# rvp-group/srrg2_proslam

Hardware: AMD Instinct MI355X
Metric: tracked frames/sec on KITTI-00 stereo (1241x376, ~2k kp); SE(3) vs ref (higher is better)
Workload: dtype u64 popcount (Hamming) + f32 (projection, Jacobians, 6x6 normal equations)

## Files before the change

srrg2_proslam_amd/csrc/align.hip:

```cpp
#include "prs_device.h"
#include "prs_host.h"
#include "prs_se3.h"

#include <math.h>
#include <string.h>

#include <type_traits>
#include <vector>

namespace prs {

constexpr int kAlignThreads = 256;
constexpr int kTerms        = 29;
constexpr uint32_t kNoneU32 = 0xffffffffu;
constexpr float kFltMax     = 3.402823466e+38f;

typedef unsigned int au32x4 __attribute__((ext_vector_type(4)));

struct AlignShared {
  float X[16];
  float A[16];
  float Sinv[16];
  float T[16];
  float Tprev[16];
// ... 971 lines not shown
          if (bind) {
            const uint32_t wsum = wave_inclusive_scan_dpp((uint32_t) msum), wabs = wave_inclusive_scan_dpp((uint32_t) mabs);
            const bool winexact = __ballot(inexact) != 0ull;
            if (lane == 63) {
              atomicAdd(&dsum[0], (int) wsum);
              atomicAdd(&dsum[1], (int) wabs);
              if (winexact) {
                dsum[2] = 1;
              }
            }
          }
          __syncthreads();
          if (sh.error) {
            break;
          }
          {
            const int chunk_r = (R + T) / T, chunk_c = (g.ncells + T) / T;
            uint32_t sum_r = 0, sum_c = 0;
            for (int j = 0; j < chunk_r; ++j) {
              const int r = tid * chunk_r + j;
              sum_r += r <= R ? hist_row[r] : 0u;
            }
            for (int j = 0; j < chunk_c; ++j) {
              const int r = tid * chunk_c + j;
              sum_c += r <= g.ncells ? hist_cell[r] : 0u;
            }
            const uint32_t incl_r = wave_inclusive_scan_dpp(sum_r), incl_c = wave_inclusive_scan_dpp(sum_c);
            if (lane == 63) {
              sh.wave_tot[wave]          = (int) incl_r;
              sh.wave_tot[kWaves + wave] = (int) incl_c;
            }
            if (bind && tid == T - 64) {
              const bool exact = !dsum[2] && dsum[1] < (1 << 24);
              const float acc  = exact ? (float) dsum[0] * 0.0625f : serial_float_sum(disp, nF);
              sh.mean_disp     = nF > 0 ? acc / (float) (size_t) nF : 0.0f;
            }
            __syncthreads();
            uint32_t run_r = incl_r - sum_r, run_c = incl_c - sum_c;
#pragma unroll
            for (int w = 0; w < kWaves; ++w) {
              run_r += w < wave ? (uint32_t) sh.wave_tot[w] : 0u;
              run_c += w < wave ? (uint32_t) sh.wave_tot[kWaves + w] : 0u;
            }
            for (int j = 0; j < chunk_r; ++j) {
              const int r = tid * chunk_r + j;
              if (r <= R) {
                rowfirst[r] = (uint16_t) run_r;
                run_r += hist_row[r];
              }
            }
            for (int j = 0; j < chunk_c; ++j) {
              const int r = tid * chunk_c + j;
              if (r <= g.ncells) {
                cellstart[r] = (uint16_t) run_c;
                run_c += hist_cell[r];
              }
            }
          }
          __syncthreads();
          for (int i = tid; i < nF; i += T) {
            bucket[rowfirst[rowcol[i] & 0xffffu] + slot[i]] = (uint16_t) i;
          }
          __syncthreads();
          for (int i = tid; i < nF; i += T) {
            const uint32_t rc = rowcol[i];
            const int row = (int) (rc & 0xffffu), col = (int) (rc >> 16);
            const int s = rowfirst[row], e = rowfirst[row + 1];
            int rank = 0;
            for (int j = s; j < e; ++j) {
              rank += bucket[j] < (uint16_t) i ? 1 : 0;
            }
            const int canon = s + rank;
            int cxi         = col >> g.cell_sx;
            cxi             = cxi < g.cell_ncx ? cxi : g.cell_ncx - 1;
            db[cellstart[(row >> g.cell_sy) * g.cell_ncx + cxi] + cslot[i]] = make_uint2(rc, (uint32_t) i | ((uint32_t) canon << 16));
            inv[canon]                                                      = (uint16_t) i;
          }
          if (tid == 0) {
            db[nF] = make_uint2(0x7fff7fffu, 0xffffffffu);
          }
          __syncthreads();
          db_built = true;
          if (split_search && g.dbcache) {
            const uint4* src = reinterpret_cast<const uint4*>(smem + g.off_db);
            uint4* dst       = reinterpret_cast<uint4*>(g.dbcache + (size_t) frame * g.db_blob);
            for (int i = tid; i < (int) (g.db_blob >> 4); i += T) {
              dst[i] = src[i];
            }
            if (tid == 0) {
              ctl->db_ready = 1;
            }
          }
        }

        SUB_ACC(acc_db);
        const int rad = (int) sh.radius;
        {
          const int tid = cold_copy(tid_hot);
          for (int i = tid; i < nF; i += T) {
            bestkey[i] = kNoneU32;
            second[i]  = kNoneU32;
          }
          if (lattice) {
            if (stage_rows) {
              au32x4* rows = split_search && g.rowcache ? g.rowcache + (size_t) frame * 2 * (size_t) g.max_fixed : nullptr;
              for (int pos = tid; pos < nF; pos += T) {
                const int fi    = (int) (db[pos].y & 0xffffu);
                const au32x4 lo = gfd[2 * fi], hi = gfd[2 * fi + 1];
                fdesc[pos]      = lo;
                fdesc_hi[pos]   = hi;
                if (rows) {
                  rows[pos]               = lo;
                  rows[g.max_fixed + pos] = hi;
                }
              }
            }
          } else {
            for (int i = tid; i < 2 * nF; i += T) {
              (i & 1 ? fdesc_hi : fdesc)[i >> 1] = gfd[i];
            }
            for (int i = tid; i < nF; i += T) {
              const float4 c = gfix[i];
              fuv[i]         = make_float2(c.x, c.y);
            }
          }
          if (stype == PRS_SEARCH_CIRCLE) {
            for (int i = tid; i < 2 * rad + 1 && i < g.lut_cap; i += T) {
              const int h = i - rad;
              lut[i]      = (uint16_t) (isqrt_exact(rad * rad - h * h) + 1);
            }
          }
        }
        __syncthreads();
        SUB_ACC(acc_pass2);
        {
          const float W0 = sh.W[0], W1 = sh.W[1], W2 = sh.W[2], W3 = sh.W[3];
          const float W4 = sh.W[4], W5 = sh.W[5], W6 = sh.W[6], W7 = sh.W[7];
          const float W8 = sh.W[8], W9 = sh.W[9], W10 = sh.W[10], W11 = sh.W[11];
          const float cols = (float) g.f.projector.canvas_cols, rows = (float) g.f.projector.canvas_rows;
          const float max_dd = g.f.maximum_descriptor_distance;
          const float r2f    = (float) (sh.radius * sh.radius);
          const int rad2     = rad * rad;
          const int irrelevant = irrelevant_distance(sh.dd, g.f.maximum_distance_ratio_to_second_best);
          const int prune_at   = (lattice && irrelevant > 0 && irrelevant <= 54 && !g.no_prefilter && !sh.no_prune) ? irrelevant : 0;
          const bool circle_exact = rad < 8192 && R + rad < 32000 && (g.cell_ncx << g.cell_sx) + rad < 32000;
          int projected      = 0;
          const bool q_on   = kReuse && split_search && g.qcache != nullptr && prune_at > 0;
          const int q_tag   = q_on ? (prune_at | ((prune_at <= g.narrow_prefilter_limit ? 3 : 4) << 8)) : 0;
          const bool q_read = q_on && (sh.q_tag & 0xffff) == q_tag;
          au32x4* const qc  = q_on ? g.qcache + mbase : nullptr;
          if (kReuse && split_search && tid == 0) {
            sh.q_tag = (sh.q_tag & 0xffff) | (q_tag << 16);
          }
          auto query = [&](const int m, const float4 p, au32x4 q0, au32x4 q1, auto first_pass_tag) {
            constexpr bool FIRST_PASS = decltype(first_pass_tag)::value;
            au32x4 ent = {0u, 0u, 0u, 0u};
            if (FIRST_PASS) {
              ent = qc[m];
            }
            const float x = ((W0 * p.x + W1 * p.y) + W2 * p.z) + W3;
            const float y = ((W4 * p.x + W5 * p.y) + W6 * p.z) + W7;
            const float z = ((W8 * p.x + W9 * p.y) + W10 * p.z) + W11;
            uint2 cd      = make_uint2(kNoneU32, kNoneU32);
            bool visible  = !(z < g.f.projector.range_min || z > g.f.projector.range_max);
            float u = 0.0f, v = 0.0f;
            if (visible) {
              const float hx = g.f.projector.fx * x + g.f.projector.cx * z;
              const float hy = g.f.projector.fy * y + g.f.projector.cy * z;
              u              = hx / z;
              v              = hy / z;
              visible        = !(u < 0.0f || u >= cols || v < 0.0f || v >= rows);
            }
            if (!FIRST_PASS && SPLIT && SLOTS == 4) {
              asm volatile("" : "+v"(q0), "+v"(q1));
            }
            if (visible) {
              if (!FIRST_PASS) {
                ++projected;
              }
              bool hit = false, cached = false;
              uint32_t bestk = kNoneU32, seck = kNoneU32;
              int row = 0, col = 0, rmin = 0, rmax = 0, cmin = 0, cmax = 0;
              int r0, r1, cb0, cb1;
              if (lattice) {
                row  = (int) (int16_t) roundf(v);
                col  = (int) (int16_t) roundf(u);
                rmin = (int) (int16_t) (row - rad);
                rmax = (int) (int16_t) (row + rad + 1);
                cmin = (int) (int16_t) (col - rad - 1);
                cmax = (int) (int16_t) (col + rad + 1);
                r0   = rmin;
                r1   = rmax - 1;
                cb0  = col - rad;
                cb1  = col + rad;
              } else {
                const KdNode* nodes        = reinterpret_cast<const KdNode*>(db);
                const uint16_t* leaf_start = cellstart + 2;
                int code                   = (int) reinterpret_cast<const short*>(cellstart)[0];
                while (code >= 0) {
                  const KdNode nd = nodes[code];
                  code            = (int) nd.child[kd_side(nd, u, v) < 0.0f ? 0 : 1];
                }
                const int leaf = ~code;
                for (int o = leaf_start[leaf]; o < (int) leaf_start[leaf + 1]; ++o) {
                  const int fi   = inv[o];
                  const float2 c = fuv[fi];
                  const float du = c.x - u, dv = c.y - v;
                  if (du * du + dv * dv < r2f) {
                    const uint32_t d   = (uint32_t) hamming_regs(fdesc[fi], fdesc_hi[fi], q0, q1);
                    const uint32_t key = (float) d < max_dd ? ((d << 16) | (uint32_t) fi) : kNoneU32;
                    bestk              = key < bestk ? key : bestk;
                  }
                }
                r0 = 1;
                r1 = cb0 = cb1 = 0;
              }
              r0  = (lattice && r0 < 0) ? 0 : r0;
              r1  = r1 > R - 1 ? R - 1 : r1;
              cb0 = cb0 < 0 ? 0 : cb0;
              const int colmax = (g.cell_ncx << g.cell_sx) - 1;
              cb1 = cb1 > colmax ? colmax : cb1;
              if (r0 <= r1 && cb0 <= cb1) {
                const int cx0 = cb0 >> g.cell_sx, cx1 = cb1 >> g.cell_sx;
                const uint32_t query_rc = ((uint32_t) row & 0xffffu) | ((uint32_t) col << 16);
                auto accepts_circle = [&](const uint2 e) -> bool {
                  typedef short i16x2 __attribute__((ext_vector_type(2)));
                  const i16x2 d = __builtin_bit_cast(i16x2, e.x) - __builtin_bit_cast(i16x2, query_rc);
                  return __builtin_amdgcn_sdot2(d, d, 0, false) <= rad2;
                };
                auto accepts_any = [&](const uint2 e) -> bool {
                  const int drow = (int) (int16_t) (e.x & 0xffffu);
                  const int dcol = (int) (int16_t) (e.x >> 16);
                  if (drow < rmin || drow >= rmax) {
                    return false;
                  } else if (stype == PRS_SEARCH_SQUARE) {
                    return dcol > cmin && dcol < cmax;
                  } else if (stype == PRS_SEARCH_CIRCLE) {
                    const int h     = drow - row;
                    const int li    = h + rad;
                    const int width = li < g.lut_cap ? (int) lut[li] : isqrt_exact(rad * rad - h * h) + 1;
                    return dcol > col - width && dcol < col + width;
                  } else {
                    int width = (int) (int16_t) (drow - rmin + 1);
                    if (width > (int) (int16_t) rad) {
                      width = (int) (int16_t) (rmax - drow);
                    }
                    return dcol > col - width && dcol < col + width;
                  }
                };
                const bool lean_circle = stype == PRS_SEARCH_CIRCLE && circle_exact;
                auto score_at = [&](const int p) {
                  const uint32_t ey = db[p].y;
                  const uint32_t d  = (uint32_t) hamming_regs(fdesc[p], fdesc_hi[p], q0, q1);
                  const uint32_t key = (d << 16) | (ey >> 16);
                  const uint32_t hi  = key > bestk ? key : bestk;
                  seck               = hi < seck ? hi : seck;
                  bestk              = key < bestk ? key : bestk;
                };
                typedef __attribute__((address_space(3))) unsigned char lds_byte;
                const uint32_t fd_lds = (uint32_t) (uintptr_t) (lds_byte*) fdesc;
                auto scan = [&](auto accepts, auto pruned_tag) {
                  constexpr int WORDS = decltype(pruned_tag)::value;
                  constexpr bool PRUNED = WORDS != 0;
                  const uint16_t* cs = cellstart + (r0 >> g.cell_sy) * g.cell_ncx + cx0;
                  const int width    = cx1 + 1 - cx0;
                  int rows_left      = (r1 >> g.cell_sy) - (r0 >> g.cell_sy) + 1;
                  int pos = 0, seg1 = 0;
                  int n_surv = 0;
                  for (;;) {
                    if (pos >= seg1) {
                      if (rows_left <= 0) {
                        break;
                      }
                      pos  = cs[0];
                      seg1 = cs[width];
                      cs += g.cell_ncx;
                      --rows_left;
                    }
                    if (pos < seg1) {
                      if (PRUNED) {
                        au32x4 la, lb;
                        asm volatile("ds_read_b128 %0, %2\n\tds_read_b128 %1, %2 offset:16\n\ts_waitcnt lgkmcnt(0)"
                                     : "=&v"(la), "=&v"(lb)
                                     : "v"(fd_lds + 16u * (uint32_t) pos));
                        const bool hit_a = (WORDS == 3 ? hamming_96(la, q0) : hamming_half(la, q0)) < prune_at;
                        const bool hit_b = (WORDS == 3 ? hamming_96(lb, q0) : hamming_half(lb, q0)) < prune_at;
                        if (hit_a) {
                          surv[n_surv & (kSurvivors - 1)] = (uint16_t) pos;
                          ++n_surv;
                        }
                        if (hit_b) {
                          surv[n_surv & (kSurvivors - 1)] = (uint16_t) (pos + 1);
                          ++n_surv;
                        }
                      } else {
                        const unsigned long long wa = reinterpret_cast<const unsigned long long*>(db)[pos];
                        const unsigned long long wb = reinterpret_cast<const unsigned long long*>(db)[pos + 1];
                        const uint2 ea = make_uint2((uint32_t) wa, (uint32_t) (wa >> 32)), eb = make_uint2((uint32_t) wb, (uint32_t) (wb >> 32));
                        const bool in_a = accepts(ea);
                        const bool in_b = (pos + 1 < seg1) & accepts(eb);
                        if (in_a) {
                          score_at(pos);
                        }
                        if (in_b) {
                          score_at(pos + 1);
                        }
                      }
                      pos += 2;
                    }
                  }
                  return n_surv;
                };
                auto scan_pattern = [&](auto pruned_tag) {
                  return lean_circle ? scan(accepts_circle, pruned_tag) : scan(accepts_any, pruned_tag);
                };
                auto settle = [&](const int n_surv) {
                  for (int i = 0; i < n_surv; ++i) {
                    const int p = (int) surv[i];
                    bool seen   = false;
                    for (int j = 0; j < i; ++j) {
                      seen = seen | ((int) surv[j] == p);
                    }
                    if (!seen && (lean_circle ? accepts_circle(db[p]) : accepts_any(db[p]))) {
                      score_at(p);
                    }
                  }
                };
                if (FIRST_PASS) {
                  const int cy0 = r0 >> g.cell_sy, cy1 = r1 >> g.cell_sy;
                  hit = ent.y != 0u && ent.y <= (uint32_t) kSurvivors + 1u && cx0 >= (int) (ent.x & 0xffu) && cx1 <= (int) ((ent.x >> 8) & 0xffu) && cy0 >= (int) ((ent.x >> 16) & 0xffu) &&
                        cy1 <= (int) (ent.x >> 24);
                  if (hit && ent.y > 1u) {
                    q0 = gmd[2 * m];
                    q1 = gmd[2 * m + 1];
                    *reinterpret_cast<uint2*>(surv) = make_uint2(ent.z, ent.w);
                    settle((int) ent.y - 1);
                  }
                } else if (prune_at > 0) {
                  const int n_surv = (prune_at <= g.narrow_prefilter_limit) ? scan_pattern(std::integral_constant<int, 3>{}) : scan_pattern(std::integral_constant<int, 4>{});
                  if (n_surv > kSurvivors) {
                    atomicAdd(&sh.n_overflow, 1);
                    scan_pattern(std::integral_constant<int, 0>{});
                  } else {
                    settle(n_surv);
                    if (q_on) {
                      const uint2 kept = *reinterpret_cast<const uint2*>(surv);
                      qc[m]  = au32x4{(uint32_t) cx0 | ((uint32_t) cx1 << 8) | ((uint32_t) (r0 >> g.cell_sy) << 16) | ((uint32_t) (r1 >> g.cell_sy) << 24),
                                      (uint32_t) n_surv + 1u, kept.x, kept.y};
                      cached = true;
                    }
                  }
                } else {
                  scan_pattern(std::integral_constant<int, 0>{});
                }
              }
              if (FIRST_PASS) {
                if (!hit) {
                  g.missq[mbase + (size_t) atomicAdd(&sh.q_miss, 1)] = (uint16_t) m;
                  bestk = kNoneU32;
                } else {
                  ++projected;
                }
              } else if (q_on && !cached) {
                const uint32_t none = (uint32_t) cold_copy(0);
                qc[m]               = au32x4{none, none, none, none};
              }
              if (bestk != kNoneU32) {
                cd.x = (lattice ? (uint32_t) inv[bestk & 0xffffu] : (bestk & 0xffffu)) | ((bestk >> 16) << 16);
                if (lattice && seck != kNoneU32) {
                  cd.y = (uint32_t) inv[seck & 0xffffu] | ((seck >> 16) << 16);
                }
              }
              auto emit = [&](const uint32_t c, const uint32_t tag) {
                const uint32_t f   = c & 0xffffu;
                const uint32_t key = ((c >> 16) << 17) | ((uint32_t) m << 1) | tag;
                const uint32_t old = atomicMin(&bestkey[f], key);
                if (old != kNoneU32) {
                  atomicMin(&second[f], (old > key ? old : key) >> 17);
                }
              };
              if (cd.x != kNoneU32) {
                emit(cd.x, 0u);
              }
              if (cd.y != kNoneU32) {
                emit(cd.y, 1u);
              }
            } else if (FIRST_PASS ? ent.y != 0u : q_on) {
              const uint32_t none = (uint32_t) cold_copy(0);
              qc[m]               = au32x4{none, none, none, none};
            }
          };
          constexpr int kPre = SPLIT ? 1 : 4;
          if constexpr (!kReuse) {
            for (int m0 = tid; m0 < nM; m0 += kPre * T) {
              float4 pre_p[kPre];
              au32x4 pre_q0[kPre], pre_q1[kPre];
#pragma unroll
              for (int qi = 0; qi < kPre; ++qi) {
                const int mm = m0 + qi * T < nM ? m0 + qi * T : m0;
                pre_p[qi]    = gmov[mm];
                pre_q0[qi]   = gmd[2 * mm];
                pre_q1[qi]   = gmd[2 * mm + 1];
              }
#pragma unroll
              for (int qi = 0; qi < kPre; ++qi) {
                const int m = m0 + qi * T;
                if (m >= nM) {
                  continue;
                }
                query(m, pre_p[qi], pre_q0[qi], pre_q1[qi], std::false_type{});
              }
            }
          } else {
            static_assert(kPre == 1, "the search half fetches one query at a time");
            int n_query = nM;
            if (q_read) {
              for (int m = tid; m < nM; m += T) {
                query(m, gmov[m], au32x4{0u, 0u, 0u, 0u}, au32x4{0u, 0u, 0u, 0u}, std::true_type{});
              }
              __syncthreads();
              SUB_ACC(acc_lin);
              n_query = sh.q_miss;
            }
            for (int i = tid; i < n_query; i += T) {
              const int m = q_read ? (int) g.missq[mbase + (size_t) i] : i;
              query(m, gmov[m], gmd[2 * m], gmd[2 * m + 1], std::false_type{});
            }
          }
          if (projected) {
            atomicAdd(&sh.n_projected, projected);
          }
        }
        __syncthreads();
        SUB_ACC(acc_search);
        const int f_tid = kReuse ? cold_copy(tid_hot) : tid, f_lane = kReuse ? (f_tid & 63) : lane, f_wave = kReuse ? (f_tid >> 6) : wave;
        {
          const int tid = f_tid, lane = f_lane, wave = f_wave;
          const float ratio = g.f.maximum_distance_ratio_to_second_best;
          const float dd    = sh.dd;
          int base          = 0;
          constexpr int kWaves = T / 64;
          static_assert(2 * kWaves <= 16, "AlignShared::wave_tot holds the wave totals of two chunks");
          for (int f0 = 0; f0 < nF; f0 += 2 * T) {
            if (f0 != 0) {
              __syncthreads();
            }
            bool acc[2];
            int pre[2];
#pragma unroll
            for (int k = 0; k < 2; ++k) {
              const int f = f0 + k * T + tid;
              acc[k]      = false;
              if (f < nF) {
                const uint32_t bk = bestkey[f];
                if (bk != kNoneU32) {
                  const float resp = (float) (bk >> 17);
                  const uint32_t s = second[f];
                  const float fs   = s == kNoneU32 ? kFltMax : (float) s;
                  acc[k] = resp < dd && resp / fs < ratio && (bk & 1u) == 0u;
                }
              }
              const unsigned long long bal = __ballot(acc[k]);
              pre[k]                       = __popcll(bal & ((1ull << lane) - 1ull));
              if (lane == 0) {
                sh.wave_tot[k * kWaves + wave] = __popcll(bal);
              }
            }
            __syncthreads();
            int wbase[2] = {0, 0};
            int run      = base;
#pragma unroll
            for (int j = 0; j < 2 * kWaves; ++j) {
              if (j == wave) {
                wbase[0] = run;
              }
              if (j == kWaves + wave) {
                wbase[1] = run;
              }
              run += sh.wave_tot[j];
            }
            base = run;
#pragma unroll
            for (int k = 0; k < 2; ++k) {
              const int f = f0 + k * T + tid;
              if (f < nF) {
                second[f] = acc[k] ? (uint32_t) (wbase[k] + pre[k]) : kNoneU32;
              }
            }
          }
          if (tid == 0) {
            sh.n_filtered = base;
          }
        }
        if (tid == 0) {
          if (sh.n_projected == 0) {
            sh.flags |= PRS_WARN_NO_PROJECTION;
          }
          if (8 * sh.n_overflow > sh.n_projected) {
            sh.no_prune = 1;
          }
          if (kReuse && split_search) {
            const int tag_now = sh.q_tag >> 16;
            if (tag_now != 0 && (sh.q_tag & 0xffff) == tag_now) {
              atomicAdd(&ctl->q_hits, sh.n_projected - sh.q_miss);
              atomicAdd(&ctl->q_misses, sh.q_miss);
            }
            sh.q_tag = tag_now;
          }
          const float matching_ratio = (float) sh.n_filtered / (float) (size_t) nF;
          sh.decision                = kDecisionCommit;
          if (matching_ratio < g.f.minimum_matching_ratio) {
            sh.flags |= PRS_WARN_LOW_RATIO;
            if (sh.radius < g.f.maximum_search_radius_pixels || sh.dd > g.f.minimum_descriptor_distance) {
              sh.radius = g.f.maximum_search_radius_pixels;
              sh.dd     = g.f.minimum_descriptor_distance;
              sh.flags |= PRS_WARN_RETRIED;
              if (matching_ratio == 0.0f) {
                sh.flags |= PRS_WARN_TRACK_LOST;
                se3_identity(sh.T);
                sh.it = 0;
              } else {
                ++sh.it;
              }
              sh.decision = kDecisionRetry;
            }
          }
          if (sh.decision == kDecisionCommit) {
            sh.n_corr       = sh.n_filtered;
            sh.corr_changed = 1;
            if (sh.change_norm < g.f.maximum_estimate_change_norm_for_convergence &&
                sh.it > g.f.minimum_number_of_iterations) {
              sh.converged = 1;
              if (matching_ratio > g.f.minimum_matching_ratio) {
                const unsigned long long reduced = sh.radius - g.f.search_radius_step_size_pixels;
                sh.radius = reduced > g.f.minimum_search_radius_pixels ? reduced : g.f.minimum_search_radius_pixels;
                const float increased = sh.dd + g.f.descriptor_distance_step_size_pixels;
                sh.dd = increased < g.f.maximum_descriptor_distance ? increased : g.f.maximum_descriptor_distance;
              }
            }
            ++sh.it;
          }
        }
        __syncthreads();
        if (sh.decision == kDecisionRetry) {
          continue;
        }
        SUB_ACC(acc_filter);
        for (int f = cold_copy(tid_hot); f < nF; f += T) {
          const uint32_t slot = second[f];
          if (slot != kNoneU32) {
            const uint32_t bk = bestkey[f];
            const int m       = (int) ((bk >> 1) & 0xffffu);
            prs_corr cr;
            cr.fixed_idx  = f;
            cr.moving_idx = m;
            cr.response   = (float) (bk >> 17);
            gcorr[slot]   = cr;
            if (g.mode == PRS_MODE_ALIGN) {
              cfix[slot] = gfix[f];
              cmov[slot] = gmov[m];
            }
          }
        }
        if (!split_search || g.stamps) {
          __syncthreads();
        }
        SUB_ACC(acc_commit);
        break;
      }
      if (sh.error) {
        break;
      }
      if (tid == 0 && sh.n_corr == 0) {
        sh.flags |= PRS_WARN_NO_MATCHES;
      }
      if (!split_search) {
        __syncthreads();
      }
    }
// ... 827 lines not shown
#define GN(...) PRS_VARIANT("prs::", gn_kernel, AlignArgs, __VA_ARGS__)
static const Variant<AlignArgs> kAlignVariants[] = {
    AK(256, false, -1, 4),
    AK(512, true, 2, 8), AK(512, true, 2, 4), AK(512, true, 1, 8), AK(512, true, 1, 4), AK(512, true, 3, 8), AK(512, true, 3, 4), AK(512, true, 0, 4),
    GN(4, 4, false, 4, 1, 1), GN(4, 4, false, 4, 1, 0), GN(8, 4, false, 4, 1, 1), GN(8, 4, false, 4, 1, 0),
    GN(4, 4, false, 4, 4, 2), GN(4, 4, false, 4, 4, 0), GN(4, 4, false, 4, 4, 1), GN(4, 3, true, 4, 4, 0), GN(4, 0, true, 4, 4, 0),
    GN(8, 4, false, 3, 5, 2), GN(8, 4, false, 3, 5, 0), GN(8, 4, false, 3, 5, 1), GN(8, 3, true, 4, 4, 0), GN(8, 0, true, 4, 4, 0),
};
#undef AK
#undef GN
static_assert(kAlignThreads == 256 && kSearchThreads == 512 && kGnLdsSlots == 4 && PRS_SEARCH_KDTREE == 0 && PRS_SEARCH_SQUARE == 1 && PRS_SEARCH_CIRCLE == 2 &&
                PRS_SEARCH_RHOMBUS == 3 && PRS_FACTOR_DEPTH == 3 && PRS_FACTOR_STEREO == 4,
              "kAlignVariants spells these as literals");

const char* align_kernel_name(int index) {
  return index >= 0 && index < (int) (sizeof(kAlignVariants) / sizeof(kAlignVariants[0])) ? kAlignVariants[index].name : nullptr;
}

struct AlignPlan : Plan {
  AlignArgs g = {}, gs = {};
  bool split = false, stamps_split = false;
  bool reuse = false;
  bool lone = false, five = false, fast = false, plain = false, mprior = false, depth = false;
};

static AlignPlan align_plan(const prs_pcf_params& finder, const prs_aligner_params& aligner, const prs_align_batch& batch, int mode, const DispatchEnv& env) {
  AlignPlan p;
  if (mode < PRS_MODE_ALIGN || mode > PRS_MODE_LINEARIZE) {
    p.refuse(PRS_ERR_UNSUPPORTED, "prs_align_batch_run: unknown mode");
    return p;
  }
  if (batch.batch <= 0) {
    return p;
  }
  if (batch.fixed_stride <= 0 || batch.fixed_stride > 32767 || batch.moving_stride <= 0 || batch.moving_stride > 65535) {
    p.refuse(PRS_ERR_UNSUPPORTED, "prs_align_batch_run: fixed_stride must be in [1,32767], moving_stride in [1,65535]");
    return p;
  }
  if (finder.projector.canvas_rows <= 0 || finder.projector.canvas_rows > 8192 || finder.projector.canvas_cols <= 0 ||
      finder.projector.canvas_cols > 32767) {
    p.refuse(PRS_ERR_UNSUPPORTED, "prs_align_batch_run: projector canvas must be within 32767 x 8192");
    return p;
  }
  if (finder.maximum_search_radius_pixels > 16383 || finder.search_type < PRS_SEARCH_KDTREE || finder.search_type > PRS_SEARCH_RHOMBUS) {
    p.refuse(PRS_ERR_UNSUPPORTED, "prs_align_batch_run: search radius > 16383 px or unknown search type");
    return p;
  }
  if (aligner.factor_type != PRS_FACTOR_MONO && aligner.factor_type != PRS_FACTOR_DEPTH && aligner.factor_type != PRS_FACTOR_STEREO) {
    p.refuse(PRS_ERR_UNSUPPORTED, "prs_align_batch_run: factor_type must be 2, 3 or 4");
    return p;
  }
  if ((aligner.kernel_weight_form != PRS_KERNEL_WEIGHT_INV_CHI && aligner.kernel_weight_form != PRS_KERNEL_WEIGHT_TAU_OVER_CHI) ||
      (aligner.damping_form != PRS_DAMPING_DIAG && aligner.damping_form != PRS_DAMPING_IDENTITY) ||
      (aligner.translation_weight_form != PRS_TRANSLATION_WEIGHT_OFFSET && aligner.translation_weight_form != PRS_TRANSLATION_WEIGHT_CLAMP)) {
    p.refuse(PRS_ERR_UNSUPPORTED, "prs_align_batch_run: unknown kernel_weight_form / damping_form / translation_weight_form");
    return p;
  }
  AlignArgs& g = p.g;
  g.mode       = mode;
  g.rows_table = finder.projector.canvas_rows;
  const int max_fixed = batch.max_fixed > 0 && batch.max_fixed < batch.fixed_stride ? batch.max_fixed : batch.fixed_stride;
  g.max_fixed       = max_fixed;
  const uint32_t nf = (uint32_t) max_fixed;
  const uint32_t R  = (uint32_t) g.rows_table;
  uint32_t lut_cap  = 2u * (uint32_t) finder.maximum_search_radius_pixels + 1u;
  if (lut_cap > 2048u) {
    lut_cap = 2048u;
  }
  g.lut_cap = (int) lut_cap;
  int sy = 4, sx = 4;
  auto cells_of = [&](int shift_y, int shift_x, int& ncy, int& ncx) {
    ncy = ((int) R + (1 << shift_y) - 1) >> shift_y;
    ncx = (finder.projector.canvas_cols + (1 << shift_x) - 1) >> shift_x;
    return ncy * ncx;
  };
  int ncy = 0, ncx = 0;
  while (cells_of(sy, sx, ncy, ncx) > 2048) {
    if (ncy > ncx) {
      ++sy;
    } else {
      ++sx;
    }
  }
  g.cell_sy  = sy;
  g.cell_sx  = sx;
  g.cell_ncy = ncy;
  g.cell_ncx = ncx;
  g.ncells   = ncy * ncx;
  const bool kdtree         = finder.search_type == PRS_SEARCH_KDTREE;
  const uint32_t cs_entries = kdtree && nf + 4u > (uint32_t) g.ncells + 2u ? nf + 4u : (uint32_t) g.ncells + 2u;
  auto carve = [&](AlignArgs& g, bool with_operands) -> size_t {
    uint32_t off = 0;
    g.off_db       = off; off = align_up16(off + (nf + 1) * 8);
    g.off_inv      = off; off = align_up16(off + nf * 2);
    g.off_cellstart = off; off = align_up16(off + cs_entries * 2);
    g.off_cfix     = off; off = align_up16(off + (with_operands ? nf * 16 : 0));
    g.off_cmov     = off; off = align_up16(off + (with_operands ? nf * 16 : 0));
    g.off_cls      = off; off = align_up16(off + (with_operands ? nf : 0));
    g.off_sh       = off; off = align_up16(off + (uint32_t) sizeof(AlignShared));
    g.off_u        = off;
    uint32_t u = off;
    g.off_fdesc  = u; u = align_up16(u + nf * 32);
    g.off_fuv    = u; u = align_up16(u + (kdtree ? nf * 8 : 0));
    g.off_best   = u; u = align_up16(u + nf * 4);
    g.off_second = u; u = align_up16(u + nf * 4);
    g.off_lut    = u; u = align_up16(u + lut_cap * 2);
    g.off_surv   = u; u = align_up16(u + (uint32_t) (with_operands ? kAlignThreads : kSearchThreads) * (uint32_t) g.surv_slots * 2);
    g.off_terms = off;
    uint32_t terms_bytes       = kTerms * kAlignThreads * 4;
    const uint32_t build_bytes = (nf + 40) * 4 + (R + 2 + (uint32_t) g.ncells + 2) * 4 + nf * 4 + 16 + (nf + 2) * 2 * 3 + (R + 2) * 2 + 16;
    if (build_bytes > terms_bytes) {
      terms_bytes = build_bytes;
    }
    const uint32_t kd_bytes = (uint32_t) kd_open_capacity((int) nf) * (40 + 7 * 4) + (nf + 2) * 2 * 3 + 64;
    if (kdtree && kd_bytes > terms_bytes) {
      terms_bytes = kd_bytes;
    }
    const uint32_t t_end = align_up16(off + terms_bytes);
    return u > t_end ? u : t_end;
  };
  g.surv_slots     = 4;
  const size_t lds = carve(g, true);
  if (lds > 160 * 1024) {
    p.refuse(PRS_ERR_UNSUPPORTED, "prs_align_batch_run: fixed cloud does not fit the 160 KiB LDS (lower max_fixed)");
    return p;
  }
  if (max_fixed >= (int) kClsOutUnit) {
    p.refuse(PRS_ERR_UNSUPPORTED, "prs_align_batch_run: max_fixed must be below 2048");
    return p;
  }
  p.stamps_split = env.stamps && env.stamps_split;
  p.split        = mode == PRS_MODE_ALIGN && !env.fused_align && max_fixed <= kGnThreads * kGnSlots && (!env.stamps || p.stamps_split);
  if (!p.split) {
    p.add(find_variant(kAlignVariants, {kAlignThreads, 0, -1, 4}), batch.batch, 1, kAlignThreads, lds);
    return p;
  }
  AlignArgs& gs = p.gs;
  gs            = g;
  gs.mode       = kModeSplitSearch;
  gs.surv_slots = 8;
  size_t lds_search = carve(gs, false);
  gs.surv_slots     = 4;
  {
    const size_t lds4 = carve(gs, false);
    if ((160u * 1024u) / lds_search == (160u * 1024u) / lds4 && !kdtree) {
      gs.surv_slots = 8;
      lds_search    = carve(gs, false);
    } else {
      lds_search = lds4;
    }
  }
  gs.db_blob = align_up16(gs.off_cellstart + cs_entries * 2) - gs.off_db;
  p.add(find_variant(kAlignVariants, {kSearchThreads, 1, finder.search_type, gs.surv_slots}), batch.batch, 1, kSearchThreads, lds_search);
  p.reuse = !env.no_search_reuse && !kdtree && gs.surv_slots == 4 && ncx <= 256 && ncy <= 256;
  p.fast = aligner.factor_type == PRS_FACTOR_STEREO && !aligner.keep_only_inlier_correspondences && aligner.kernel_weight_form == PRS_KERNEL_WEIGHT_INV_CHI &&
           aligner.damping_form == PRS_DAMPING_DIAG && aligner.translation_weight_form == PRS_TRANSLATION_WEIGHT_OFFSET;
  p.lone = p.fast && batch.batch <= 2 * env.cus && !env.no_lone_gn;
  p.five = p.fast && !p.lone && max_fixed > 4 * 128;
  const bool lean = !batch.prior && !aligner.with_sensor && !aligner.enable_inlier_only_runs;
  p.plain  = lean && !aligner.enable_motion_prior;
  p.mprior = lean && aligner.enable_motion_prior;
  p.depth = aligner.factor_type == PRS_FACTOR_DEPTH && aligner.kernel_weight_form == PRS_KERNEL_WEIGHT_INV_CHI && aligner.damping_form == PRS_DAMPING_DIAG;
  const int slots = max_fixed <= 4 * 128 ? 4 : 8, lds_slots = p.five ? 3 : kGnLdsSlots;
  const int gn    = p.fast ? find_variant(kAlignVariants, {slots, PRS_FACTOR_STEREO, 0, lds_slots, p.lone ? 1 : (p.five ? 5 : 4),
                                                           p.plain ? 1 : (p.mprior && !p.lone ? 2 : 0)})
                           : find_variant(kAlignVariants, {slots, p.depth ? PRS_FACTOR_DEPTH : 0, 1, kGnLdsSlots, 4, 0});
  p.add(gn, batch.batch, 1, kGnThreads, gn_lds_bytes(lds_slots));
  return p;
}

int align_batch_launch(prs_context* ctx, const prs_pcf_params* finder, const prs_aligner_params* aligner, const prs_align_batch* batch, int mode, int rounds) {
  if (ctx->align_job && static_cast<SplitJob*>(ctx->align_job)->active) {
    return ctx_fail(ctx, PRS_ERR_UNSUPPORTED, "prs_align_batch_*: the previous batch of this context has not been finished (prs_align_batch_finish)");
  }
  if (!finder || !aligner || !batch || !batch->fixed || !batch->fixed_desc || !batch->n_fixed || !batch->moving ||
      !batch->moving_desc || !batch->n_moving || !batch->state || !batch->X || !batch->corr || !batch->n_corr || !batch->result) {
    return ctx_fail(ctx, PRS_ERR_NULL, "prs_align_batch_run: fixed, moving, correspondences, state or result not set");
  }
  const AlignPlan plan = align_plan(*finder, *aligner, *batch, mode, dispatch_env(ctx));
  if (plan.status != PRS_OK) {
    return ctx_fail(ctx, plan.status, plan.message);
  }
  if (plan.n_launches == 0) {
    return PRS_OK;
  }
  unsigned long long* stamps = ctx_stamps(ctx, (size_t) batch->batch * 16 * sizeof(unsigned long long));
  auto with_inputs = [&](AlignArgs a) {
    a.f          = *finder;
    a.a          = *aligner;
    a.b          = *batch;
    a.no_prefilter = ctx->no_prefilter ? 1 : 0;
    a.narrow_prefilter_limit = ctx->prefilter_96_limit;
    a.prior_mean = batch->prior_mean;
    a.stamps     = stamps;
    return a;
  };
  AlignArgs g        = with_inputs(plan.g);
  hipStream_t stream = ctx_stream(ctx);
  hipError_t e;
  if (!plan.split) {
    const Plan::Launch& l = plan.launch[0];
    auto kernel = kAlignVariants[l.kernel].fn;
    e           = hipFuncSetAttribute(reinterpret_cast<const void*>(kernel), hipFuncAttributeMaxDynamicSharedMemorySize, (int) l.lds);
    if (e != hipSuccess) {
      return ctx_fail_hip(ctx, e, "prs_align_batch_run attribute");
    }
    hipLaunchKernelGGL(kernel, dim3(l.grid_x), dim3(l.block), l.lds, stream, g);
    if (ctx->align_job) {
      static_cast<SplitJob*>(ctx->align_job)->last = false;
    }
    e = hipGetLastError();
    if (e != hipSuccess) {
      return ctx_fail_hip(ctx, e, "prs_align_batch_run launch");
    }
    if (g.stamps) {
      ctx_report_stamps(ctx, batch->batch, 10, "align (fused, 256 threads): finder | linearize + in-wave reduction | cross-wave sum | GN solve || of finder: lattice build | projection+search | staging (keys, fixed rows -> LDS) | filter | commit");
    }
    return PRS_OK;
  }
  const Plan::Launch &ls = plan.launch[0], &lg = plan.launch[1];
  SplitJob* job = static_cast<SplitJob*>(ctx->align_job);
  if (!job) {
    job                 = new SplitJob();
    ctx->align_job      = job;
    ctx->align_job_free = [](void* p) { delete static_cast<SplitJob*>(p); };
  }
  const int max_fixed    = g.max_fixed;
  const size_t ops_bytes = (size_t) batch->batch * (size_t) max_fixed * 2 * sizeof(float4);
  const size_t ctl_bytes = (size_t) batch->batch * sizeof(FrameCtl) + 256;
  unsigned char* small   = static_cast<unsigned char*>(job->buffer(stream, 0, ctl_bytes));
  g.ops                  = static_cast<float4*>(job->buffer(stream, 1, ops_bytes));
  if (!small || !g.ops) {
    return ctx_fail(ctx, PRS_ERR_HIP, "prs_align_batch_run: split-pipeline scratch allocation failed");
  }
  g.pending = reinterpret_cast<int*>(small);
  g.ctl     = reinterpret_cast<FrameCtl*>(small + 256);
  AlignArgs gs = with_inputs(plan.gs);
  gs.ops       = g.ops;
  gs.pending   = g.pending;
  gs.ctl       = g.ctl;
  gs.dbcache   = static_cast<unsigned char*>(job->buffer(stream, 2, (size_t) batch->batch * gs.db_blob));
  if (!gs.dbcache) {
    return ctx_fail(ctx, PRS_ERR_HIP, "prs_align_batch_run: lattice cache allocation failed");
  }
  if (finder->search_type != PRS_SEARCH_KDTREE) {
    gs.rowcache = static_cast<au32x4*>(job->buffer(stream, 3, (size_t) batch->batch * (size_t) max_fixed * 2 * sizeof(au32x4)));
    if (!gs.rowcache) {
      return ctx_fail(ctx, PRS_ERR_HIP, "prs_align_batch_run: descriptor row cache allocation failed");
    }
  }
  if (plan.reuse) {
    const size_t queries = (size_t) batch->batch * (size_t) batch->moving_stride;
    gs.qcache            = static_cast<au32x4*>(job->buffer(stream, 4, queries * sizeof(au32x4)));
    gs.missq             = gs.qcache ? static_cast<uint16_t*>(job->buffer(stream, 5, queries * sizeof(uint16_t))) : nullptr;
    if (!gs.missq) {
      (void) hipGetLastError();
      gs.qcache = nullptr;
    }
  }
  e = hipFuncSetAttribute(reinterpret_cast<const void*>(kAlignVariants[ls.kernel].fn), hipFuncAttributeMaxDynamicSharedMemorySize, (int) ls.lds);
  if (e != hipSuccess) {
    return ctx_fail_hip(ctx, e, "prs_align_batch_run attribute");
  }
  hipLaunchKernelGGL(split_init_kernel, dim3((batch->batch + 255) / 256), dim3(256), 0, stream, g.ctl, batch->result, g.pending, batch->batch);
  job->active      = true;
  job->stream      = stream;
  job->capture_stream = stream;
  job->g           = g;
  job->gs          = gs;
  job->search      = kAlignVariants[ls.kernel].fn;
  job->gn          = kAlignVariants[lg.kernel].fn;
  job->last        = true;
  job->lds_search  = ls.lds;
  job->lds_gn      = lg.lds;
  job->total       = 0;
  job->limit       = 2 * (aligner->max_iterations + inlier_run_length(*aligner)) + 8;
  job->ev_used     = 0;
  job->rounds_timed = 0;
  job->stamps      = plan.stamps_split && stamps;
  job->enqueued    = rounds > 0 ? rounds : 5;
  return split_rounds(ctx, job, job->enqueued);
}

static int split_rounds(prs_context* ctx, SplitJob* job, int rounds) {
  hipStream_t stream = job->stream;
  auto tick = [&]() {
    if (ctx->timing && job->ev_used < 3 * 64) {
      if (!ctx->timing_ev[job->ev_used]) {
        (void) hipEventCreate(&ctx->timing_ev[job->ev_used]);
      }
      (void) hipEventRecord(ctx->timing_ev[job->ev_used], stream);
      ++job->ev_used;
    }
  };
  const int batch = job->g.b.batch;
  for (int r = 0; r < rounds; ++r) {
    (void) hipMemsetAsync(job->g.pending, 0, sizeof(int), stream);
    tick();
    hipLaunchKernelGGL(job->search, dim3(batch), dim3(kSearchThreads), job->lds_search, stream, job->gs);
    tick();
    if (job->stamps) {
      ctx_report_stamps(ctx, batch, 10, "search launch (split): - | query-cache pass | - | - || lattice build | projection+search (behind a cache pass: the scan of its queue) | staging (keys, fixed rows -> LDS) | filter | commit");
    }
    hipLaunchKernelGGL(job->gn, dim3(batch), dim3(kGnThreads), job->lds_gn, stream, job->g);
    tick();
    ++job->total;
  }
// ... 161 lines not shown
```

Before: 1.893 million.

## Cache survivor Hamming distances in query cache to skip descriptor reloads on hits

The per-query cache entry now packs up to four survivor indices together with their Hamming distances, so the cached pass no longer reloads the query descriptors or recomputes popcounts and only re-checks geometric acceptance. The cached pass also prefetches two queries' points and cache entries per thread before processing them. Loop-invariant values are pinned to scalar registers with empty asm. Reuse is now restricted to fewer than 2048 fixed points so indices fit in 11 bits. The cost is more packing work when the cache is written and a narrower set of cases where reuse is enabled.

```diff
diff --git a/srrg2_proslam_amd/csrc/align.hip b/srrg2_proslam_amd/csrc/align.hip
--- a/srrg2_proslam_amd/csrc/align.hip
+++ b/srrg2_proslam_amd/csrc/align.hip
@@ -1147,12 +1147,8 @@
           if (kReuse && split_search && tid == 0) {
             sh.q_tag = (sh.q_tag & 0xffff) | (q_tag << 16);
           }
-          auto query = [&](const int m, const float4 p, au32x4 q0, au32x4 q1, auto first_pass_tag) {
+          auto query = [&](const int m, const float4 p, au32x4 q0, au32x4 q1, const au32x4 ent, auto first_pass_tag) {
             constexpr bool FIRST_PASS = decltype(first_pass_tag)::value;
-            au32x4 ent = {0u, 0u, 0u, 0u};
-            if (FIRST_PASS) {
-              ent = qc[m];
-            }
             const float x = ((W0 * p.x + W1 * p.y) + W2 * p.z) + W3;
             const float y = ((W4 * p.x + W5 * p.y) + W6 * p.z) + W7;
             const float z = ((W8 * p.x + W9 * p.y) + W10 * p.z) + W11;
@@ -1244,13 +1240,16 @@
                   }
                 };
                 const bool lean_circle = stype == PRS_SEARCH_CIRCLE && circle_exact;
-                auto score_at = [&](const int p) {
-                  const uint32_t ey = db[p].y;
-                  const uint32_t d  = (uint32_t) hamming_regs(fdesc[p], fdesc_hi[p], q0, q1);
+                auto take = [&](const uint32_t d, const uint32_t ey) {
                   const uint32_t key = (d << 16) | (ey >> 16);
                   const uint32_t hi  = key > bestk ? key : bestk;
                   seck               = hi < seck ? hi : seck;
                   bestk              = key < bestk ? key : bestk;
+                };
+                auto score_at = [&](const int p) {
+                  const uint32_t ey = db[p].y;
+                  const uint32_t d  = (uint32_t) hamming_regs(fdesc[p], fdesc_hi[p], q0, q1);
+                  take(d, ey);
                 };
                 typedef __attribute__((address_space(3))) unsigned char lds_byte;
                 const uint32_t fd_lds = (uint32_t) (uintptr_t) (lds_byte*) fdesc;
@@ -1260,6 +1259,11 @@
                   const uint16_t* cs = cellstart + (r0 >> g.cell_sy) * g.cell_ncx + cx0;
                   const int width    = cx1 + 1 - cx0;
                   int rows_left      = (r1 >> g.cell_sy) - (r0 >> g.cell_sy) + 1;
+                  int ncx            = g.cell_ncx;
+                  uint32_t fd        = fd_lds;
+                  if constexpr (kReuse) {
+                    asm volatile("" : "+s"(ncx), "+s"(fd));
+                  }
                   int pos = 0, seg1 = 0;
                   int n_surv = 0;
                   for (;;) {
@@ -1269,7 +1273,7 @@
                       }
                       pos  = cs[0];
                       seg1 = cs[width];
-                      cs += g.cell_ncx;
+                      cs += ncx;
                       --rows_left;
                     }
                     if (pos < seg1) {
@@ -1277,7 +1281,7 @@
                         au32x4 la, lb;
                         asm volatile("ds_read_b128 %0, %2\n\tds_read_b128 %1, %2 offset:16\n\ts_waitcnt lgkmcnt(0)"
                                      : "=&v"(la), "=&v"(lb)
-                                     : "v"(fd_lds + 16u * (uint32_t) pos));
+                                     : "v"(fd + 16u * (uint32_t) pos));
                         const bool hit_a = (WORDS == 3 ? hamming_96(la, q0) : hamming_half(la, q0)) < prune_at;
                         const bool hit_b = (WORDS == 3 ? hamming_96(lb, q0) : hamming_half(lb, q0)) < prune_at;
                         if (hit_a) {
@@ -1310,26 +1314,53 @@
                   return lean_circle ? scan(accepts_circle, pruned_tag) : scan(accepts_any, pruned_tag);
                 };
                 auto settle = [&](const int n_surv) {
+                  unsigned long long packed = 0ull;
+                  uint32_t last = 0u, n = 0u;
                   for (int i = 0; i < n_surv; ++i) {
                     const int p = (int) surv[i];
                     bool seen   = false;
                     for (int j = 0; j < i; ++j) {
                       seen = seen | ((int) surv[j] == p);
                     }
-                    if (!seen && (lean_circle ? accepts_circle(db[p]) : accepts_any(db[p]))) {
-                      score_at(p);
+                    if constexpr (kReuse) {
+                      if (!seen) {
+                        const uint2 e    = db[p];
+                        const uint32_t d = (uint32_t) hamming_regs(fdesc[p], fdesc_hi[p], q0, q1);
+                        last = (uint32_t) p | (d << 11);
+                        packed |= (unsigned long long) last << (20u * n);
+                        ++n;
+                        if (lean_circle ? accepts_circle(e) : accepts_any(e)) {
+                          take(d, e.y);
+                        }
+                      }
+                    } else {
+                      if (!seen && (lean_circle ? accepts_circle(db[p]) : accepts_any(db[p]))) {
+                        score_at(p);
+                      }
                     }
                   }
+                  const uint32_t fourth = n == 4u ? last : 0u;
+                  return make_uint3(((uint32_t) packed & 0xfffffu) | ((n + 1u) << 20), ((uint32_t) (packed >> 20) & 0xfffffu) | ((fourth & 0x7ffu) << 20),
+                                    ((uint32_t) (packed >> 40) & 0xfffffu) | ((fourth >> 11) << 20));
                 };
                 if (FIRST_PASS) {
                   const int cy0 = r0 >> g.cell_sy, cy1 = r1 >> g.cell_sy;
-                  hit = ent.y != 0u && ent.y <= (uint32_t) kSurvivors + 1u && cx0 >= (int) (ent.x & 0xffu) && cx1 <= (int) ((ent.x >> 8) & 0xffu) && cy0 >= (int) ((ent.x >> 16) & 0xffu) &&
+                  const uint32_t code = ent.y >> 20;
+                  hit = code != 0u && code <= (uint32_t) kSurvivors + 1u && cx0 >= (int) (ent.x & 0xffu) && cx1 <= (int) ((ent.x >> 8) & 0xffu) && cy0 >= (int) ((ent.x >> 16) & 0xffu) &&
                         cy1 <= (int) (ent.x >> 24);
-                  if (hit && ent.y > 1u) {
-                    q0 = gmd[2 * m];
-                    q1 = gmd[2 * m + 1];
-                    *reinterpret_cast<uint2*>(surv) = make_uint2(ent.z, ent.w);
-                    settle((int) ent.y - 1);
+                  if (hit && code > 1u) {
+#pragma unroll
+                    for (int i = 0; i < 4; ++i) {
+                      if ((uint32_t) i + 1u < code) {
+                        const uint32_t w  = i == 0 ? ent.y : (i == 1 ? ent.z : ent.w);
+                        const uint32_t sp = i < 3 ? (w & 0x7ffu) : ((ent.z >> 20) & 0x7ffu);
+                        const uint32_t sd = i < 3 ? ((w >> 11) & 0x1ffu) : (ent.w >> 20);
+                        const uint2 e     = db[sp];
+                        if (lean_circle ? accepts_circle(e) : accepts_any(e)) {
+                          take(sd, e.y);
+                        }
+                      }
+                    }
                   }
                 } else if (prune_at > 0) {
                   const int n_surv = (prune_at <= g.narrow_prefilter_limit) ? scan_pattern(std::integral_constant<int, 3>{}) : scan_pattern(std::integral_constant<int, 4>{});
@@ -1337,11 +1368,10 @@
                     atomicAdd(&sh.n_overflow, 1);
                     scan_pattern(std::integral_constant<int, 0>{});
                   } else {
-                    settle(n_surv);
+                    const uint3 kept = settle(n_surv);
                     if (q_on) {
-                      const uint2 kept = *reinterpret_cast<const uint2*>(surv);
                       qc[m]  = au32x4{(uint32_t) cx0 | ((uint32_t) cx1 << 8) | ((uint32_t) (r0 >> g.cell_sy) << 16) | ((uint32_t) (r1 >> g.cell_sy) << 24),
-                                      (uint32_t) n_surv + 1u, kept.x, kept.y};
+                                      kept.x, kept.y, kept.z};
                       cached = true;
                     }
                   }
@@ -1403,15 +1433,30 @@
                 if (m >= nM) {
                   continue;
                 }
-                query(m, pre_p[qi], pre_q0[qi], pre_q1[qi], std::false_type{});
+                query(m, pre_p[qi], pre_q0[qi], pre_q1[qi], au32x4{0u, 0u, 0u, 0u}, std::false_type{});
               }
             }
           } else {
             static_assert(kPre == 1, "the search half fetches one query at a time");
             int n_query = nM;
             if (q_read) {
-              for (int m = tid; m < nM; m += T) {
-                query(m, gmov[m], au32x4{0u, 0u, 0u, 0u}, au32x4{0u, 0u, 0u, 0u}, std::true_type{});
+              constexpr int kQPre = 2;
+              for (int m0 = tid; m0 < nM; m0 += kQPre * T) {
+                float4 pre_p[kQPre];
+                au32x4 pre_e[kQPre];
+#pragma unroll
+                for (int qi = 0; qi < kQPre; ++qi) {
+                  const int mm = m0 + qi * T < nM ? m0 + qi * T : m0;
+                  pre_p[qi]    = gmov[mm];
+                  pre_e[qi]    = qc[mm];
+                }
+#pragma unroll
+                for (int qi = 0; qi < kQPre; ++qi) {
+                  const int m = m0 + qi * T;
+                  if (m < nM) {
+                    query(m, pre_p[qi], au32x4{0u, 0u, 0u, 0u}, au32x4{0u, 0u, 0u, 0u}, pre_e[qi], std::true_type{});
+                  }
+                }
               }
               __syncthreads();
               SUB_ACC(acc_lin);
@@ -1419,7 +1464,7 @@
             }
             for (int i = tid; i < n_query; i += T) {
               const int m = q_read ? (int) g.missq[mbase + (size_t) i] : i;
-              query(m, gmov[m], gmd[2 * m], gmd[2 * m + 1], std::false_type{});
+              query(m, gmov[m], gmd[2 * m], gmd[2 * m + 1], au32x4{0u, 0u, 0u, 0u}, std::false_type{});
             }
           }
           if (projected) {
@@ -2553,7 +2598,7 @@
   }
   gs.db_blob = align_up16(gs.off_cellstart + cs_entries * 2) - gs.off_db;
   p.add(find_variant(kAlignVariants, {kSearchThreads, 1, finder.search_type, gs.surv_slots}), batch.batch, 1, kSearchThreads, lds_search);
-  p.reuse = !env.no_search_reuse && !kdtree && gs.surv_slots == 4 && ncx <= 256 && ncy <= 256;
+  p.reuse = !env.no_search_reuse && !kdtree && gs.surv_slots == 4 && ncx <= 256 && ncy <= 256 && max_fixed < 2048;
   p.fast = aligner.factor_type == PRS_FACTOR_STEREO && !aligner.keep_only_inlier_correspondences && aligner.kernel_weight_form == PRS_KERNEL_WEIGHT_INV_CHI &&
            aligner.damping_form == PRS_DAMPING_DIAG && aligner.translation_weight_form == PRS_TRANSLATION_WEIGHT_OFFSET;
   p.lone = p.fast && batch.batch <= 2 * env.cus && !env.no_lone_gn;
```

Result: faster. 1.949 million (median of 6 runs) (+3.0%).
